# KlrShaK/opencv-SimpleSLAM

Hardware: AMD Instinct MI355X
Metric: frames/sec ALIKED+LightGlue @1241x376 (higher is better)
Workload: dtype f32 (contractions: f16 hi/lo split operands, f32 accumulate; 3 MFMA per product, 2 in attention's P.V = precision 'f16x3p1', the default since r05: profiles/r05_flip_soak.md, r06_flip_soak.md); 1 GPU; C2/C4: synthetic 1241x376x3 uint8 frame stream, ALIKED-n16 extract + LightGlue match (t-1,t), 2048 kpts/frame, min_conf 0.7, random-init weights; inputs resident in HBM before the timed region, features and matches left on the device (the `pcie` leg times the same pipeline with per-round H2D of the frames and D2H of {count, pairs}); max_kpts=2048, lightglue_layers_executed=9, pairs_per_lightglue_launch=8, frames_per_aliked_launch=8

## Files before the change

opencv-simpleslam_amd/csrc/al_plan.hpp:

```cpp
#pragma once
#include <algorithm>
#include <cstddef>
#include <cstdio>

namespace sslam {

constexpr int AL_LONG_SIDE = 1024;
constexpr int AL_PAD_DIV = 32;
constexpr int MAX_FRAMES = 16;
constexpr int B1_SW = 30;
constexpr int B2_SW = 30;
constexpr int DCN3_CS = 1;
constexpr int DCN4_CS = 4;
constexpr int AGG_PRE = 13;
constexpr int ST_W = 32, ST_H = 8;
constexpr int NHALO = 10;
constexpr int NW_R = 48, NW_OW = 64 - 2 * NHALO, NW_OH = NW_R - 2 * NHALO;
constexpr int HBINS = 4096;
constexpr int COLLECT_PPT = 16;
constexpr int SEL_CAP = 8192;
constexpr int EDGE_CAP = 2048;
constexpr int CAND_CAP = 1024 * 1024;
constexpr int REFINE_KPB = 32;
constexpr int SDDH_KSPLIT = 4;

constexpr int al_cdiv(int a, int b) { return (a + b - 1) / b; }

struct Dims {
    int H, W, C;
    int h, w;
    int Hp, Wp;
    int pl, pt;
};

enum class ALAggTile { T64x64, T64x128 };

struct ALPlan {
    int F, KF;
    int blur, ky, kx;
    float sy, sx;
    Dims d;
    int to_float_gx, pad_gx;
    int b1_strips, b1_nblk, b1_hs, b1_nb;
    int b2_strips, b2_nblk, b2_hs, b2_nb, b2_waves, b2_gx;
    int H2, W2, HW2, H3, W3, HW3, H4, W4, HW4;
    int pool3_gx, pool4_gx;
    int off3_gx, dcn3_gx, off4_gx, dcn4_gx;
    float mo3, mo4, mo;
    int gate2_gx, gate3_gx, gate4_gx, gate34_gx;
    float sy2, sx2, sy8, sx8, sy32, sx32;
    int agg_pre_gx;
    int tail_gx, tail_gy;
    int nbx, nby, n_tiles, nms_gx;
    int npx, collect_gx;
    ALAggTile agg_tile;
    float scale_x, scale_y;
};

inline ALPlan al_plan(int H, int W, int C, int F) {
    ALPlan p{};
    p.F = F; p.KF = SDDH_KSPLIT * F;
    Dims& d = p.d;
    d.H = H; d.W = W; d.C = C;
    const double ar = (double)W / (double)H;
    if (ar > 1.0) { d.h = (int)(AL_LONG_SIDE / ar); d.w = AL_LONG_SIDE; }
    else { d.h = AL_LONG_SIDE; d.w = (int)(AL_LONG_SIDE * ar); }
    const double fy = (double)H / d.h, fx = (double)W / d.w;
    p.blur = (fy > fx ? fy : fx) > 1.0;
    const double sgy = (fy - 1.0) / 2.0 > 0.001 ? (fy - 1.0) / 2.0 : 0.001, sgx = (fx - 1.0) / 2.0 > 0.001 ? (fx - 1.0) / 2.0 : 0.001;
    p.sy = (float)sgy; p.sx = (float)sgx;
    const double ksy = 2.0 * 2 * sgy, ksx = 2.0 * 2 * sgx;
    p.ky = (int)(ksy > 3 ? ksy : 3); p.kx = (int)(ksx > 3 ? ksx : 3);
    if (p.ky % 2 == 0) ++p.ky;
    if (p.kx % 2 == 0) ++p.kx;
    const int pad_h = (((d.h / AL_PAD_DIV) + 1) * AL_PAD_DIV - d.h) % AL_PAD_DIV;
    const int pad_w = (((d.w / AL_PAD_DIV) + 1) * AL_PAD_DIV - d.w) % AL_PAD_DIV;
    d.Hp = d.h + pad_h; d.Wp = d.w + pad_w; d.pl = pad_w / 2; d.pt = pad_h / 2;
    const int Hp = d.Hp, Wp = d.Wp;

// ... 10 lines not shown
    p.b2_waves = p.b2_strips * p.b2_nb * F;
    p.b2_gx = al_cdiv(p.b2_waves, 4);
    p.H3 = Hp / 8; p.W3 = Wp / 8; p.HW3 = p.H3 * p.W3;
    p.H4 = Hp / 32; p.W4 = Wp / 32; p.HW4 = p.H4 * p.W4;
    p.pool3_gx = al_cdiv(32 * p.HW3, 256); p.pool4_gx = al_cdiv(64 * p.HW4, 256);
    p.off3_gx = al_cdiv(p.W3, 32); p.dcn3_gx = DCN3_CS * al_cdiv(p.W3, 32);
    p.off4_gx = al_cdiv(p.W4, 32); p.dcn4_gx = DCN4_CS * al_cdiv(p.W4, 32);
    p.mo3 = (float)(p.H3 > p.W3 ? p.H3 : p.W3) / 4.0f;
    p.mo4 = (float)(p.H4 > p.W4 ? p.H4 : p.W4) / 4.0f;
    p.gate2_gx = al_cdiv(p.HW2, 256); p.gate3_gx = al_cdiv(32 * p.HW3, 256); p.gate4_gx = al_cdiv(32 * p.HW4, 256);
    p.gate34_gx = p.gate3_gx + p.gate4_gx;
    auto step = [](int full, int S) { return (float)(full / S - 1) / (float)(full - 1); };
    p.sy2 = step(Hp, 2); p.sx2 = step(Wp, 2); p.sy8 = step(Hp, 8); p.sx8 = step(Wp, 8);
    p.sy32 = step(Hp, 32); p.sx32 = step(Wp, 32);
    p.agg_pre_gx = al_cdiv(p.HW2 + p.HW3 + p.HW4, 256);
    p.tail_gx = al_cdiv(Wp, ST_W); p.tail_gy = al_cdiv(Hp, ST_H);
    p.nbx = al_cdiv(d.w, NW_OW); p.nby = al_cdiv(d.h, NW_OH); p.n_tiles = p.nbx * p.nby;
    p.nms_gx = al_cdiv(p.n_tiles, 4);
    p.npx = d.h * d.w;
    p.collect_gx = al_cdiv(p.npx, 256 * COLLECT_PPT);
    p.mo = (float)(d.h > d.w ? d.h : d.w) / 4.0f;
    p.agg_tile = F >= 4 ? ALAggTile::T64x128 : ALAggTile::T64x64;
    p.scale_x = (float)d.w / (float)W; p.scale_y = (float)d.h / (float)H;
    return p;
}

enum class ALRefusal { None, Size, Frames, Blur };
inline ALRefusal al_refusal(const ALPlan& p, int Hp_cap, int Wp_cap, int max_frames, char* msg, size_t n) {
    const Dims& d = p.d;
    if (!(d.Hp <= Hp_cap && d.Wp <= Wp_cap && d.h >= 8 && d.w >= 8)) {
        snprintf(msg, n, "sslam_aliked: network size %dx%d outside the instance capacity %dx%d", d.Hp, d.Wp, Hp_cap, Wp_cap);
        return ALRefusal::Size;
    }
    if (!(p.F >= 1 && p.F <= max_frames)) {
        snprintf(msg, n, "sslam_aliked: %d frames, instance capacity %d", p.F, max_frames);
        return ALRefusal::Frames;
    }
    if (!(p.kx <= 31 && p.ky <= 31)) {
        snprintf(msg, n, "sslam_aliked: blur kernel too large (%d,%d)", p.kx, p.ky);
        return ALRefusal::Blur;
    }
    return ALRefusal::None;
}

struct ALKptPlan {
    int NK;
// ... 55 lines not shown
```

opencv-simpleslam_amd/csrc/aliked_kernels.hip:

```cpp
#include "common.hpp"
#include "al_plan.hpp"
#include "gemm_f32.hpp"
#include <type_traits>
#include "gemm_f16x3.hpp"

namespace {

using sslam::f32x16;
using sslam::acc_row;
using sslam::GemmSmem;
using sslam::GemmA;
using sslam::gemm_mainloop;
using sslam::Dims;
using sslam::MAX_FRAMES; using sslam::B1_SW; using sslam::B2_SW; using sslam::DCN3_CS; using sslam::DCN4_CS; using sslam::AGG_PRE;
using sslam::ST_W; using sslam::ST_H; using sslam::NHALO; using sslam::NW_R; using sslam::NW_OW; using sslam::NW_OH; using sslam::HBINS;
using sslam::COLLECT_PPT; using sslam::SEL_CAP; using sslam::EDGE_CAP; using sslam::REFINE_KPB; using sslam::SDDH_KSPLIT;

constexpr float SELU_SCALE = 1.0507009873554804934193349852946f;
constexpr float SELU_ALPHA = 1.6732632423543772848170429916717f;
__device__ __forceinline__ float selu(float x) {
    return SELU_SCALE * (x > 0.0f ? x : SELU_ALPHA * (__expf(x) - 1.0f));
}

__device__ __forceinline__ float selu_precise(float x) {
// ... 22 lines not shown
    using B = std::conditional_t<std::is_const_v<T>, const char, char>;
    return reinterpret_cast<T*>(reinterpret_cast<B*>(p) + (size_t)f * fs);
}
struct Tile3 { int x, y, z; };
__device__ __forceinline__ Tile3 xcd_band() {
    const unsigned nx = gridDim.x, ny = gridDim.y, per = nx * ny;
    if ((per & 7u) == 0u) {
        const unsigned L = blockIdx.x + nx * blockIdx.y;
        const unsigned g = (L & 7u) * (per >> 3) + (L >> 3);
        return Tile3{(int)(g % nx), (int)(g / nx), (int)blockIdx.z};
    }
    return Tile3{(int)blockIdx.x, (int)blockIdx.y, (int)blockIdx.z};
}
template <typename T> __device__ __forceinline__ T* fsh0(T* p, int f, size_t fs) {
    return p ? fsh(p, f, fs) : nullptr;
}
template <typename T> __device__ __forceinline__ T& at_b(T* base, unsigned byte_off) {
    using B = std::conditional_t<std::is_const_v<T>, const char, char>;
    return *reinterpret_cast<T*>(reinterpret_cast<B*>(base) + byte_off);
}
struct FrameIn { const uint8_t* img[MAX_FRAMES]; };
struct FrameOut { float* xy[MAX_FRAMES]; float* desc[MAX_FRAMES]; float* score[MAX_FRAMES]; int32_t* n[MAX_FRAMES]; };

__global__ void al_to_float_kernel(FrameIn srcs, float* __restrict__ dst, Dims d,
                                   const float* __restrict__ gx, int kx, int blur, size_t fs) {
    const uint8_t* __restrict__ src = srcs.img[blockIdx.z];
    dst = fsh(dst, blockIdx.z, fs);
    const int x = blockIdx.x * blockDim.x + threadIdx.x, y = blockIdx.y;
    if (x >= d.W) return;
#pragma unroll
    for (int c = 0; c < 3; ++c) {
        const int sc = d.C == 1 ? 0 : 2 - c;
        float v;
        if (!blur) {
            v = (float)src[((size_t)y * d.W + x) * d.C + sc] / 255.0f;
        } else {
            v = 0.0f;
            const int r = kx / 2;
#pragma unroll 8
            for (int k = 0; k < kx; ++k) {
                int xx = x + k - r;
                xx = xx < 0 ? -xx : (xx >= d.W ? 2 * d.W - 2 - xx : xx);
                v += gx[k] * ((float)src[((size_t)y * d.W + xx) * d.C + sc] / 255.0f);
            }
        }
        dst[((size_t)c * d.H + y) * d.W + x] = v;
    }
}

__global__ void al_resize_pad_kernel(const float* __restrict__ src, float* __restrict__ img, Dims d,
                                     const float* __restrict__ gy, int ky, int blur, size_t fs) {
    const Tile3 tb = xcd_band();
    src = fsh(src, tb.z, fs); img = fsh(img, tb.z, fs);
    const int xp = tb.x * blockDim.x + threadIdx.x, yp = tb.y;
    if (xp >= d.Wp) return;
    const int y = min(max(yp - d.pt, 0), d.h - 1), x = min(max(xp - d.pl, 0), d.w - 1);
    const float sy_ = (float)d.H / (float)d.h, sx_ = (float)d.W / (float)d.w;
    float fy = sy_ * ((float)y + 0.5f) - 0.5f, fx = sx_ * ((float)x + 0.5f) - 0.5f;
    fy = fy < 0.0f ? 0.0f : fy;
    fx = fx < 0.0f ? 0.0f : fx;
    const int y0 = (int)fy, x0 = (int)fx;
    const int y1 = y0 + (y0 < d.H - 1), x1 = x0 + (x0 < d.W - 1);
    const float ly = fy - (float)y0, lx = fx - (float)x0, hy = 1.0f - ly, hx = 1.0f - lx;
#pragma unroll
    for (int c = 0; c < 3; ++c) {
        const float* p = src + (size_t)c * d.H * d.W;
        float v00, v01, v10, v11;
        if (!blur) {
            v00 = p[(size_t)y0 * d.W + x0]; v01 = p[(size_t)y0 * d.W + x1];
            v10 = p[(size_t)y1 * d.W + x0]; v11 = p[(size_t)y1 * d.W + x1];
        } else {
            v00 = v01 = v10 = v11 = 0.0f;
            const int r = ky / 2;
#pragma unroll 4
            for (int k = 0; k < ky; ++k) {
                int ya = y0 + k - r, yb = y1 + k - r;
                ya = ya < 0 ? -ya : (ya >= d.H ? 2 * d.H - 2 - ya : ya);
                yb = yb < 0 ? -yb : (yb >= d.H ? 2 * d.H - 2 - yb : yb);
                const float g = gy[k];
                v00 += g * p[(size_t)ya * d.W + x0]; v01 += g * p[(size_t)ya * d.W + x1];
                v10 += g * p[(size_t)yb * d.W + x0]; v11 += g * p[(size_t)yb * d.W + x1];
            }
        }
        img[((size_t)c * d.Hp + yp) * d.Wp + xp] = hy * (hx * v00 + lx * v01) + ly * (hx * v10 + lx * v11);
    }
}

typedef float f32x4 __attribute__((ext_vector_type(4)));

__global__ void al_conv16_wfrag_kernel(const float* __restrict__ w , _Float16* __restrict__ wf, int* range_flag) {
    const int i = blockIdx.x * blockDim.x + threadIdx.x;
    if (i >= 5 * 64 * 8) return;
    const int e = i & 7, lane = (i >> 3) & 63, ks = i >> 9;
    const int kk = lane >> 4, co = lane & 15, tap = 2 * ks + (kk >> 1), ci = 8 * (kk & 1) + e;
    const float v = tap < 9 ? w[(ci * 9 + tap) * 16 + co] : 0.0f;
    _Float16 hi, lo;
    al_split_weight(v, hi, lo, range_flag);
    wf[((ks * 2 + 0) * 64 + lane) * 8 + e] = hi;
    wf[((ks * 2 + 1) * 64 + lane) * 8 + e] = lo;
}


__global__ void al_conv32p_wfrag_kernel(const float* __restrict__ w , const float* __restrict__ wd ,
                                        _Float16* __restrict__ wf, int* range_flag) {
    const int i = blockIdx.x * blockDim.x + threadIdx.x;
    if (i >= 10 * 64 * 8) return;
    const int e = i & 7, lane = (i >> 3) & 63, ks = i >> 9;
// ... 787 lines not shown
    return fmaf(t.w10, top, __fmul_rn(t.w11, bot));
}
__device__ __forceinline__ float up_eval_cl32(const float* __restrict__ p, const UpTap& t, unsigned cb) {
    return up_mix(t, at_b(p, (unsigned)t.o00 * 128u + cb), at_b(p, (unsigned)t.o01 * 128u + cb),
                  at_b(p, (unsigned)t.o10 * 128u + cb), at_b(p, (unsigned)t.o11 * 128u + cb));
}
__device__ __forceinline__ float2 feat_pair32(const Pyr& P, const float* __restrict__ rnorm, int pl, int pt,
                                              int y, int x, int lane) {
    const int yp = y + pt, xp = x + pl;
    const unsigned pix = (unsigned)(yp * P.Wp + xp);
    float a, b;
    const unsigned cb = 4u * (lane & 31);
    if (lane < 32) {
        a = at_b(P.g1cl, pix * 128u + cb);
        b = up_eval_cl32(P.g3cl, up_tap(yp, xp, P.Hp, P.Wp, 8, P.sy8, P.sx8), cb);
    } else {
        a = up_eval_cl32(P.g2cl, up_tap(yp, xp, P.Hp, P.Wp, 2, P.sy2, P.sx2), cb);
        b = up_eval_cl32(P.g4cl, up_tap(yp, xp, P.Hp, P.Wp, 32, P.sy32, P.sx32), cb);
    }
    const float r = rnorm[pix];
    return make_float2(a * r, b * r);
}

__global__ __launch_bounds__(256) void al_score_tail_kernel(const float* __restrict__ s8, int Hp, int Wp,
                                                            const float* __restrict__ w2 ,
                                                            const float* __restrict__ w4 ,
                                                            const float* __restrict__ w6 ,
                                                            float* __restrict__ score, int h, int w, int pl,
                                                            int pt, size_t fs) {
    const Tile3 tb = xcd_band();
    s8 = fsh(s8, tb.z, fs); score = fsh(score, tb.z, fs);
    __shared__ float t0[8][ST_H + 6][ST_W + 6];
    __shared__ float t1[4][ST_H + 4][ST_W + 4];
    __shared__ float t2[4][ST_H + 2][ST_W + 2];
    const int x0 = tb.x * ST_W, y0 = tb.y * ST_H;
    const size_t HW = (size_t)Hp * Wp;
    for (int i = threadIdx.x; i < 8 * (ST_H + 6) * (ST_W + 6); i += 256) {
        const int c = i / ((ST_H + 6) * (ST_W + 6)), rem = i % ((ST_H + 6) * (ST_W + 6));
        const int yy = y0 + rem / (ST_W + 6) - 3, xx = x0 + rem % (ST_W + 6) - 3;
        (&t0[0][0][0])[i] = (yy >= 0 && yy < Hp && xx >= 0 && xx < Wp) ? s8[c * HW + (size_t)yy * Wp + xx] : 0.0f;
    }
    __syncthreads();
    for (int i = threadIdx.x; i < (ST_H + 4) * (ST_W + 4); i += 256) {
        const int ly = i / (ST_W + 4), lx = i % (ST_W + 4);
        const int yy = y0 + ly - 2, xx = x0 + lx - 2;
        float a[4] = {0, 0, 0, 0};
        if (yy >= 0 && yy < Hp && xx >= 0 && xx < Wp) {
#pragma unroll 1
            for (int ci = 0; ci < 8; ++ci)
#pragma unroll
                for (int tap = 0; tap < 9; ++tap) {
                    const float v = t0[ci][ly + tap / 3][lx + tap % 3];
#pragma unroll
                    for (int o = 0; o < 4; ++o) a[o] = fmaf(v, w2[(ci * 9 + tap) * 4 + o], a[o]);
                }
            for (int o = 0; o < 4; ++o) a[o] = selu(a[o]);
        }
        for (int o = 0; o < 4; ++o) t1[o][ly][lx] = a[o];
    }
    __syncthreads();
    for (int i = threadIdx.x; i < (ST_H + 2) * (ST_W + 2); i += 256) {
        const int ly = i / (ST_W + 2), lx = i % (ST_W + 2);
        const int yy = y0 + ly - 1, xx = x0 + lx - 1;
        float a[4] = {0, 0, 0, 0};
        if (yy >= 0 && yy < Hp && xx >= 0 && xx < Wp) {
#pragma unroll 1
            for (int ci = 0; ci < 4; ++ci)
#pragma unroll
                for (int tap = 0; tap < 9; ++tap) {
                    const float v = t1[ci][ly + tap / 3][lx + tap % 3];
#pragma unroll
                    for (int o = 0; o < 4; ++o) a[o] = fmaf(v, w4[(ci * 9 + tap) * 4 + o], a[o]);
                }
            for (int o = 0; o < 4; ++o) a[o] = selu(a[o]);
        }
        for (int o = 0; o < 4; ++o) t2[o][ly][lx] = a[o];
    }
    __syncthreads();
    for (int i = threadIdx.x; i < ST_H * ST_W; i += 256) {
        const int lx = i & (ST_W - 1), ly = i / ST_W;
        const int yy = y0 + ly, xx = x0 + lx;
        float a = 0.0f;
        for (int ci = 0; ci < 4; ++ci)
            for (int tap = 0; tap < 9; ++tap) a = fmaf(t2[ci][ly + tap / 3][lx + tap % 3], w6[ci * 9 + tap], a);
        const int uy = yy - pt, ux = xx - pl;
        if (uy >= 0 && uy < h && ux >= 0 && ux < w) score[(size_t)uy * w + ux] = 1.0f / (1.0f + expf(-a));
    }
}

static_assert(NW_R <= 64 && NW_OH > 0, "a column's rows are the bits of one 64-bit word");

__device__ __forceinline__ unsigned nw_up(unsigned v) { return (unsigned)__builtin_amdgcn_update_dpp(0, (int)v, 0x138, 0xf, 0xf, true); }
__device__ __forceinline__ unsigned nw_dn(unsigned v) { return (unsigned)__builtin_amdgcn_update_dpp(0, (int)v, 0x130, 0xf, 0xf, true); }
__device__ __forceinline__ float nw_up(float v) { return __builtin_bit_cast(float, nw_up(__builtin_bit_cast(unsigned, v))); }
__device__ __forceinline__ float nw_dn(float v) { return __builtin_bit_cast(float, nw_dn(__builtin_bit_cast(unsigned, v))); }
__device__ __forceinline__ float nw_row5(float v) {
    const float l1 = fmaxf(v, nw_up(v)), l2 = fmaxf(l1, nw_up(l1));
    const float r1 = fmaxf(v, nw_dn(v)), r2 = fmaxf(r1, nw_dn(r1));
    return fmaxf(l2, r2);
}
__device__ __forceinline__ void nw_pool5(const float (&in)[NW_R], float (&v)[NW_R]) {
    float hrow[NW_R], p[NW_R], q[NW_R];
#pragma unroll
    for (int y = 0; y < NW_R; ++y) hrow[y] = nw_row5(in[y]);
#pragma unroll
    for (int y = 0; y + 1 < NW_R; ++y) p[y] = fmaxf(hrow[y], hrow[y + 1]);
#pragma unroll
    for (int y = 0; y + 3 < NW_R; ++y) q[y] = fmaxf(p[y], p[y + 2]);
// ... 605 lines not shown

struct ALConvW { const float *w, *a, *b; };
struct ALDcnW { const float *ow, *ob, *w, *a, *b; };

struct sslam_aliked {
    sslam_ctx* ctx = nullptr;
    int max_h = 0, max_w = 0, max_kpts = 0;
    int max_frames = 1;
    size_t fs = 0;
    int Hp_cap = 0, Wp_cap = 0;
    sslam::OwnedSlab slab;
    float* blob = nullptr;
    ALConvW b1c1, b1c2, b2c1, b2c2;
    const float *b2dw, *b2db;
    ALDcnW b3c1, b3c2, b4c1, b4c2;
    const float *b3dw, *b3db, *b4dw, *b4db;
    _Float16 *b3c1of, *b3c2of, *b4c1of, *b4c2of;
    _Float16 *b3c1f, *b3c2f, *b4c1f, *b4c2f;
    const float *gw1, *gw2, *gw3, *gw4;
    const float *sh0, *sh2, *sh4, *sh6;
    const float *d_ow, *d_ob, *d_w2, *d_b2, *d_sf, *d_agg;
    ALCtrl* ctrl;
    uint8_t* in_u8;
    float *fsrc, *img, *x1, *x2, *p3, *off, *t3, *x3, *p4, *t4, *x4, *g2, *g3, *g4;
    float *s8, *rnorm, *score, *nms, *bsum, *gk, *g1cl, *g2cl, *g3cl, *g4cl, *pre2, *pre3, *pre4;
    unsigned long long* cand;
    unsigned* hist;
    int cand_cap;
    int* kp_index;
    int* range_sticky;
    unsigned long long* sel_keys;
    float *kp_norm, *kp_score, *patch, *h32, *pos, *sampled, *feats, *raw;
    _Float16 *d_sf_s, *d_agg_s;
    _Float16* b2c2f;
    _Float16* b1c2f;
    _Float16* b2c1f;
    float *p3cl, *t3cl, *p4cl, *t4cl;
    float *out_xy, *out_desc, *out_score;
    int32_t* out_n;
    Dims last{};
    sslam::ALKptPlan kp{};
    bool use_graphs = false;
    sslam::GraphCache graphs;
};

namespace {

// ... 11 lines not shown
    g->b2c1 = conv(16, 32); g->b2c2 = conv(32, 32); g->b2dw = take(16 * 32); g->b2db = take(32);
    g->b3c1 = dcn(32, 64); g->b3c2 = dcn(64, 64); g->b3dw = take(32 * 64); g->b3db = take(64);
    g->b4c1 = dcn(64, 128); g->b4c2 = dcn(128, 128); g->b4dw = take(64 * 128); g->b4db = take(128);
    g->gw1 = take(16 * 32); g->gw2 = take(32 * 32); g->gw3 = take(64 * 32); g->gw4 = take(128 * 32);
    g->sh0 = take(128 * 8); g->sh2 = take(8 * 9 * 4); g->sh4 = take(4 * 9 * 4); g->sh6 = take(4 * 9);
    g->d_ow = take(32 * 1152); g->d_ob = take(32); g->d_w2 = take(32 * 32); g->d_b2 = take(32);
    g->d_sf = take(128 * 128); g->d_agg = take((size_t)128 * 2048);
    SSLAM_REQUIRE(off == n_floats, "sslam_aliked_create: weight blob has %zu floats, expected %zu", n_floats, off);
    return 0;
}

constexpr int SEL_LDS = (SEL_CAP + EDGE_CAP) * 8;

int al_enqueue(sslam_aliked* g, const sslam::ALPlan& p, const FrameIn& srcs, int n_limit, const FrameOut& outs) {
    hipStream_t s = g->ctx->stream;
    (void)hipGetLastError();
    const Dims& d = p.d;
    const sslam::ALKptPlan& k = g->kp;
    const int F = p.F, KF = p.KF, NK = k.NK;
    const size_t fs = g->fs;
    const dim3 b256(256);
    hipLaunchKernelGGL(al_reset_kernel, dim3(F), b256, 0, s, g->ctrl, g->hist, fs, g->gk, p.kx, p.sx, p.ky, p.sy);

    hipLaunchKernelGGL(al_to_float_kernel, dim3(p.to_float_gx, d.H, F), b256, 0, s, srcs, g->fsrc, d, g->gk, p.kx, p.blur, fs);
    hipLaunchKernelGGL(al_resize_pad_kernel, dim3(p.pad_gx, d.Hp, F), b256, 0, s, g->fsrc, g->img, d, g->gk + 32, p.ky, p.blur, fs);
    hipLaunchKernelGGL(al_block1_rows_kernel, dim3(p.b1_strips, p.b1_nb, F), dim3(64), 0, s, g->img, g->x1, d.Hp, d.Wp, p.b1_hs,
                       g->b1c1.w, g->b1c1.a, g->b1c1.b, g->b1c2f, g->b1c2.a, g->b1c2.b, g->ctrl, fs);
    hipLaunchKernelGGL(al_block2_rows_kernel, dim3(p.b2_gx), b256, B2_LDS, s, g->x1, g->x2, p.H2, p.W2, p.b2_hs, p.b2_nb, p.b2_strips,
                       p.b2_waves, g->b2c1f, g->b2c2f, g->b2c1.a, g->b2c1.b, g->b2db, g->b2c2.a, g->b2c2.b, g->ctrl, fs);
    const dim3 off3 = dim3(p.off3_gx, p.H3, F), dcn3 = dim3(p.dcn3_gx, p.H3, F);
    hipLaunchKernelGGL(al_avgpool_kernel, dim3(p.pool3_gx, F), b256, 0, s, g->x2, g->p3, 32, p.H2, p.W2, 4, fs, g->p3cl);
    hipLaunchKernelGGL((al_offset_conv_h_kernel<32>), off3, b256, 0, s, g->p3cl, g->off, p.H3, p.W3, g->b3c1of, g->b3c1.ob, p.mo3, g->ctrl, fs);
    hipLaunchKernelGGL((al_dcn_h_kernel<32, 64, 0, DCN3_CS>), dcn3, b256, 0, s, g->p3cl, g->off, nullptr, p.H3, p.W3, g->b3c1f, g->b3c1.b, nullptr, g->t3, g->t3cl, g->ctrl, fs);
    hipLaunchKernelGGL((al_offset_conv_h_kernel<64>), off3, b256, 0, s, g->t3cl, g->off, p.H3, p.W3, g->b3c2of, g->b3c2.ob, p.mo3, g->ctrl, fs);
    hipLaunchKernelGGL((al_dcn_h_kernel<64, 64, 32, DCN3_CS>), dcn3, b256, 0, s, g->t3cl, g->off, g->p3cl, p.H3, p.W3, g->b3c2f, g->b3c2.b, g->b3db, g->x3, nullptr, g->ctrl, fs);
    const dim3 off4 = dim3(p.off4_gx, p.H4, F), dcn4 = dim3(p.dcn4_gx, p.H4, F);
    sslam::graph_cut(s);
    hipLaunchKernelGGL(al_avgpool_kernel, dim3(p.pool4_gx, F), b256, 0, s, g->x3, g->p4, 64, p.H3, p.W3, 4, fs, g->p4cl);
    hipLaunchKernelGGL((al_offset_conv_h_kernel<64>), off4, b256, 0, s, g->p4cl, g->off, p.H4, p.W4, g->b4c1of, g->b4c1.ob, p.mo4, g->ctrl, fs);
    hipLaunchKernelGGL((al_dcn_h_kernel<64, 128, 0, DCN4_CS>), dcn4, b256, 0, s, g->p4cl, g->off, nullptr, p.H4, p.W4, g->b4c1f, g->b4c1.b, nullptr, g->t4, g->t4cl, g->ctrl, fs);
    hipLaunchKernelGGL((al_offset_conv_h_kernel<128>), off4, b256, 0, s, g->t4cl, g->off, p.H4, p.W4, g->b4c2of, g->b4c2.ob, p.mo4, g->ctrl, fs);
    hipLaunchKernelGGL((al_dcn_h_kernel<128, 128, 64, DCN4_CS>), dcn4, b256, 0, s, g->t4cl, g->off, g->p4cl, p.H4, p.W4, g->b4c2f, g->b4c2.b, g->b4db, g->x4, nullptr, g->ctrl, fs);
    hipLaunchKernelGGL(al_gate_kernel<32>, dim3(p.gate2_gx, F), b256, 0, s, g->x2, g->g2, p.HW2, g->gw2, g->g2cl, fs);
    hipLaunchKernelGGL(al_gate_small_kernel, dim3(p.gate34_gx, F), b256, 0, s, GateSmall{g->x3, g->g3, 64, p.HW3, g->gw3, g->g3cl},
                       GateSmall{g->x4, g->g4, 128, p.HW4, g->gw4, g->g4cl}, p.gate3_gx, fs);
    Pyr P{g->x1, g->g2, g->g3, g->g4, g->gw1, d.Hp, d.Wp, g->g1cl};
    P.sy2 = p.sy2; P.sx2 = p.sx2; P.sy8 = p.sy8; P.sx8 = p.sx8; P.sy32 = p.sy32; P.sx32 = p.sx32;
    P.g2cl = g->g2cl; P.g3cl = g->g3cl; P.g4cl = g->g4cl;
    P.pre2 = g->pre2; P.pre3 = g->pre3; P.pre4 = g->pre4;
    hipLaunchKernelGGL(al_agg_pre_kernel, dim3(p.agg_pre_gx, F), b256, 0, s, g->g2, g->g3, g->g4, g->sh0, g->pre2, g->pre3, g->pre4,
                       d.Hp, d.Wp, fs);
    hipLaunchKernelGGL(al_aggregate_kernel, dim3(p.pad_gx, d.Hp, F), b256, 0, s, P, g->sh0, g->s8, g->rnorm, fs);
    hipLaunchKernelGGL(al_score_tail_kernel, dim3(p.tail_gx, p.tail_gy, F), b256, 0, s, g->s8, d.Hp, d.Wp, g->sh2, g->sh4, g->sh6,
                       g->score, d.h, d.w, d.pl, d.pt, fs);
    hipLaunchKernelGGL(al_nms_wave_kernel, dim3(p.nms_gx, F), b256, 0, s, g->score, d.h, d.w, p.nbx, p.n_tiles, g->nms, g->bsum, 0.2f,
                       g->cand, g->cand_cap, g->ctrl, g->hist, fs);
    sslam::graph_cut(s);
    hipLaunchKernelGGL(al_collect_kernel, dim3(p.collect_gx, F), b256, 0, s, g->nms, p.npx, 0.0f, 1, g->bsum, p.n_tiles, g->cand,
                       g->cand_cap, g->ctrl, g->hist, fs);
    hipLaunchKernelGGL(al_select_kernel, dim3(F), dim3(1024), SEL_LDS, s, g->cand, g->cand_cap, n_limit, g->sel_keys, g->ctrl, g->hist, fs);
    hipLaunchKernelGGL(al_refine_kernel, dim3(k.refine_gx, F), b256, 0, s, g->score, d.h, d.w, g->sel_keys, g->kp_index, g->kp_norm,
                       g->kp_score, g->ctrl, fs);
    hipLaunchKernelGGL(al_patch_kernel, dim3(k.patch_gx, F), b256, 0, s, P, g->rnorm, d.pl, d.pt, d.h, d.w, g->kp_norm, g->patch, g->ctrl, fs);
    hipLaunchKernelGGL((al_gemm_kernel<64, 64, 1, 1>), dim3(1, k.rows64, KF), b256, 0, s, g->patch, 1152, g->d_ow, nullptr, 32, g->h32,
                       1, NK, 0, g->ctrl, SDDH_KSPLIT, fs);
    hipLaunchKernelGGL(al_offsets_kernel, dim3(k.offsets_gx, F), b256, 0, s, g->h32, NK, g->d_ob, g->d_w2, g->d_b2, g->kp_norm, d.h, d.w,
                       p.mo, g->pos, g->ctrl, fs);
    _Float16* sampled_h = reinterpret_cast<_Float16*>(g->sampled);
    _Float16* feats_h = reinterpret_cast<_Float16*>(g->feats);
    hipLaunchKernelGGL(al_sample_kernel, dim3(k.sample_gx, F), b256, 0, s, P, g->rnorm, d.pl, d.pt, d.h, d.w, g->pos, sampled_h,
                       k.plane, g->ctrl, fs);
    hipLaunchKernelGGL((al_gemm_h_kernel<64, 128, 1, 2, true>), dim3(1, k.rows64_x16, F), b256, 0, s, sampled_h, k.plane, 128, g->d_sf_s,
                       (size_t)128 * 128, 128, nullptr, feats_h, k.plane, 16, k.rows_x16, g->ctrl, 1, fs);
    if (p.agg_tile == sslam::ALAggTile::T64x128)
        hipLaunchKernelGGL((al_gemm_h_kernel<64, 128, 1, 2, false>), dim3(1, k.rows64, KF), b256, 0, s, feats_h, k.plane, 2048,
                           g->d_agg_s, (size_t)128 * 2048, 128, g->raw, nullptr, 0, 1, NK, g->ctrl, SDDH_KSPLIT, fs);
// ... 35 lines not shown
                  SEL_CAP);
    SSLAM_HIP_CHECK(hipSetDevice(ctx->device));
    std::unique_ptr<sslam_aliked> g(new sslam_aliked());
    g->ctx = ctx; g->max_h = max_h; g->max_w = max_w; g->max_kpts = max_kpts; g->max_frames = max_frames;
    g->kp = sslam::al_kpt_plan(max_kpts);
    g->Hp_cap = sslam::AL_LONG_SIDE + sslam::AL_PAD_DIV; g->Wp_cap = sslam::AL_LONG_SIDE + sslam::AL_PAD_DIV;
    const sslam::ALExtents e = sslam::al_extents((size_t)g->Hp_cap * g->Wp_cap, (size_t)max_h * max_w, (size_t)max_kpts);
    g->cand_cap = sslam::CAND_CAP;
    auto bind_shared = [&](sslam::Slab& A) {
        g->blob = A.take<float>(n_floats);
        g->d_sf_s = A.take<_Float16>(2 * 128 * 128); g->d_agg_s = A.take<_Float16>((size_t)2 * 128 * 2048);
        g->b2c2f = A.take<_Float16>(2 * 32 * 288);
        g->b1c2f = A.take<_Float16>(5 * 2 * 64 * 8);
        g->b2c1f = A.take<_Float16>(10 * 2 * 64 * 8);
        g->b3c1f = A.take<_Float16>((size_t)(9 * 2 + 0) * 2 * 2 * 512); g->b3c2f = A.take<_Float16>((size_t)(9 * 4 + 2) * 2 * 2 * 512);
        g->b4c1f = A.take<_Float16>((size_t)(9 * 4 + 0) * 4 * 2 * 512); g->b4c2f = A.take<_Float16>((size_t)(9 * 8 + 4) * 4 * 2 * 512);
        g->b3c1of = A.take<_Float16>(18 * 2 * 512); g->b3c2of = A.take<_Float16>(36 * 2 * 512); g->b4c1of = A.take<_Float16>(36 * 2 * 512); g->b4c2of = A.take<_Float16>(72 * 2 * 512);
        g->gk = A.take<float>(64);
        g->range_sticky = A.take<int>(4);
    };
    auto bind_frame = [&](sslam::Slab& A) {
        g->ctrl = A.take<ALCtrl>(e.ctrl);
        g->in_u8 = A.take<uint8_t>(e.in_u8);
        g->fsrc = A.take<float>(e.fsrc); g->img = A.take<float>(e.img);
        g->x1 = A.take<float>(e.x1); g->x2 = A.take<float>(e.x2);
        g->p3 = A.take<float>(e.p3); g->off = A.take<float>(e.off);
        g->t3 = A.take<float>(e.t3); g->x3 = A.take<float>(e.x3);
        g->p3cl = A.take<float>(e.p3cl); g->t3cl = A.take<float>(e.t3cl);
        g->p4cl = A.take<float>(e.p4cl); g->t4cl = A.take<float>(e.t4cl);
        g->p4 = A.take<float>(e.p4); g->t4 = A.take<float>(e.t4); g->x4 = A.take<float>(e.x4);
        g->g2 = A.take<float>(e.g2); g->g3 = A.take<float>(e.g3); g->g4 = A.take<float>(e.g4);
        g->g2cl = A.take<float>(e.g2cl); g->g3cl = A.take<float>(e.g3cl); g->g4cl = A.take<float>(e.g4cl);
        g->s8 = A.take<float>(e.s8); g->rnorm = A.take<float>(e.rnorm); g->g1cl = A.take<float>(e.g1cl);
        g->pre2 = A.take<float>(e.pre2); g->pre3 = A.take<float>(e.pre3); g->pre4 = A.take<float>(e.pre4);
        g->score = A.take<float>(e.score); g->nms = A.take<float>(e.nms); g->bsum = A.take<float>(e.bsum);
        g->cand = A.take<unsigned long long>(e.cand); g->hist = A.take<unsigned>(e.hist);
        g->kp_index = A.take<int>(e.kp_index); g->sel_keys = A.take<unsigned long long>(e.sel_keys);
        g->kp_norm = A.take<float>(e.kp_norm); g->kp_score = A.take<float>(e.kp_score);
        g->patch = A.take<float>(e.patch); g->h32 = A.take<float>(e.h32); g->pos = A.take<float>(e.pos);
        g->sampled = A.take<float>(e.sampled); g->feats = A.take<float>(e.feats);
        g->raw = A.take<float>(e.raw);
        g->out_xy = A.take<float>(e.out_xy); g->out_desc = A.take<float>(e.out_desc); g->out_score = A.take<float>(e.out_score);
        g->out_n = A.take<int32_t>(e.out_n);
    };
    sslam::Slab ms, mf;
    bind_shared(ms);
    bind_frame(mf);
// ... 192 lines not shown
```

Baseline: 1223 frames/s.

## Fuse u8-to-float blur and resize-pad into one LDS-tiled preprocess kernel; restage score tail

Replaces the separate to_float and resize_pad kernels with one tiled kernel. It stages raw uint8 rows into LDS with dword loads, applies the horizontal blur through a byte-to-float lookup table, then does the vertical blur and bilinear resize from LDS. This removes the full-resolution float intermediate (fsrc) and one launch. The score tail kernel is also reworked: LDS buffers are flattened and aliased, staging is a lane per column, and each thread computes two adjacent outputs with float2 window reads. The risks are LDS pressure from the dynamic tile size and more complex edge handling.

Result: faster. 1242 frames/s, median of 6 (+1.6%).

```diff
diff --git a/opencv-simpleslam_amd/csrc/al_plan.hpp b/opencv-simpleslam_amd/csrc/al_plan.hpp
--- a/opencv-simpleslam_amd/csrc/al_plan.hpp
+++ b/opencv-simpleslam_amd/csrc/al_plan.hpp
@@ -14,6 +14,7 @@
 constexpr int DCN4_CS = 4;
 constexpr int AGG_PRE = 13;
 constexpr int ST_W = 32, ST_H = 8;
+constexpr int PRE_LDS_MAX = 48 * 1024;
 constexpr int NHALO = 10;
 constexpr int NW_R = 48, NW_OW = 64 - 2 * NHALO, NW_OH = NW_R - 2 * NHALO;
 constexpr int HBINS = 4096;
@@ -55,6 +56,7 @@
     int npx, collect_gx;
     ALAggTile agg_tile;
     float scale_x, scale_y;
+    int pre_tw, pre_th, pre_gx, pre_gy, pre_cols, pre_rows, pre_raw, pre_lds;
 };
 
 inline ALPlan al_plan(int H, int W, int C, int F) {
@@ -111,6 +113,19 @@
     p.mo = (float)(d.h > d.w ? d.h : d.w) / 4.0f;
     p.agg_tile = F >= 4 ? ALAggTile::T64x128 : ALAggTile::T64x64;
     p.scale_x = (float)d.w / (float)W; p.scale_y = (float)d.h / (float)H;
+    {
+        static constexpr int ladder[][2] = {{64, 8}, {32, 8}, {32, 4}, {16, 4}, {16, 2}, {8, 2}, {8, 1}, {4, 1}};
+        const int rx = p.blur ? p.kx / 2 : 0, ry = p.blur ? p.ky / 2 : 0, planes = C == 1 ? 1 : 3;
+        for (const auto& t : ladder) {
+            p.pre_tw = t[0]; p.pre_th = t[1];
+            p.pre_cols = (int)(fx * (t[0] - 1)) + 4;
+            p.pre_rows = (int)(fy * (t[1] - 1)) + 4 + 2 * ry;
+            p.pre_raw = ((p.pre_cols + 2 * rx) * C + 3) / 4 * 4 + 4;
+            p.pre_lds = 256 * 4 + planes * p.pre_rows * p.pre_cols * 4 + p.pre_rows * p.pre_raw;
+            if (p.pre_lds <= PRE_LDS_MAX) break;
+        }
+        p.pre_gx = al_cdiv(Wp, p.pre_tw); p.pre_gy = al_cdiv(Hp, p.pre_th);
+    }
     return p;
 }
 
diff --git a/opencv-simpleslam_amd/csrc/aliked_kernels.hip b/opencv-simpleslam_amd/csrc/aliked_kernels.hip
--- a/opencv-simpleslam_amd/csrc/aliked_kernels.hip
+++ b/opencv-simpleslam_amd/csrc/aliked_kernels.hip
@@ -68,67 +68,150 @@
 struct FrameIn { const uint8_t* img[MAX_FRAMES]; };
 struct FrameOut { float* xy[MAX_FRAMES]; float* desc[MAX_FRAMES]; float* score[MAX_FRAMES]; int32_t* n[MAX_FRAMES]; };
 
-__global__ void al_to_float_kernel(FrameIn srcs, float* __restrict__ dst, Dims d,
-                                   const float* __restrict__ gx, int kx, int blur, size_t fs) {
-    const uint8_t* __restrict__ src = srcs.img[blockIdx.z];
-    dst = fsh(dst, blockIdx.z, fs);
-    const int x = blockIdx.x * blockDim.x + threadIdx.x, y = blockIdx.y;
-    if (x >= d.W) return;
-#pragma unroll
-    for (int c = 0; c < 3; ++c) {
-        const int sc = d.C == 1 ? 0 : 2 - c;
-        float v;
-        if (!blur) {
-            v = (float)src[((size_t)y * d.W + x) * d.C + sc] / 255.0f;
-        } else {
-            v = 0.0f;
-            const int r = kx / 2;
-#pragma unroll 8
-            for (int k = 0; k < kx; ++k) {
-                int xx = x + k - r;
-                xx = xx < 0 ? -xx : (xx >= d.W ? 2 * d.W - 2 - xx : xx);
-                v += gx[k] * ((float)src[((size_t)y * d.W + xx) * d.C + sc] / 255.0f);
+struct PreTile { int tw, th, cols, rows, raw; };
+__device__ __forceinline__ int al_reflect(int i, int n) {
+    i = i < 0 ? -i : (i >= n ? 2 * n - 2 - i : i);
+    return min(max(i, 0), n - 1);
+}
+__device__ __forceinline__ void al_src_pos(int o, int n_in, float s, int& i0, int& i1, float& l) {
+    float f = fmaf(s, __fadd_rn((float)o, 0.5f), -0.5f);
+    f = f < 0.0f ? 0.0f : f;
+    i0 = (int)f; i1 = i0 + (i0 < n_in - 1); l = __fsub_rn(f, (float)i0);
+}
+__global__ __launch_bounds__(256) void al_preprocess_kernel(FrameIn srcs, float* __restrict__ img, Dims d, const float* __restrict__ gk,
+                                                            int kx, int ky, int blur, PreTile t, size_t fs) {
+    extern __shared__ __attribute__((aligned(16))) unsigned char pre_lds[];
+    const Tile3 tb = xcd_band();
+    const uint8_t* __restrict__ src = srcs.img[tb.z];
+    img = fsh(img, tb.z, fs);
+    const int planes = d.C == 1 ? 1 : 3;
+    float* tab = reinterpret_cast<float*>(pre_lds);
+    float* hb = tab + 256;
+    uint8_t* raw = reinterpret_cast<uint8_t*>(hb + planes * t.rows * t.cols);
+    const int tid = threadIdx.x, lane = tid & 63, wv = tid >> 6;
+    const float sy_ = (float)d.H / (float)d.h, sx_ = (float)d.W / (float)d.w;
+    const int rx = blur ? kx / 2 : 0, ry = blur ? ky / 2 : 0;
+    const int xp_a = tb.x * t.tw, yp_a = tb.y * t.th;
+    const int xp_b = min(xp_a + t.tw, d.Wp) - 1, yp_b = min(yp_a + t.th, d.Hp) - 1;
+    int xlo, xhi, ylo, yhi, unused; float unused_l;
+    al_src_pos(min(max(xp_a - d.pl, 0), d.w - 1), d.W, sx_, xlo, unused, unused_l);
+    al_src_pos(min(max(xp_b - d.pl, 0), d.w - 1), d.W, sx_, unused, xhi, unused_l);
+    al_src_pos(min(max(yp_a - d.pt, 0), d.h - 1), d.H, sy_, ylo, unused, unused_l);
+    al_src_pos(min(max(yp_b - d.pt, 0), d.h - 1), d.H, sy_, unused, yhi, unused_l);
+    ylo -= ry; yhi += ry;
+    const int ncols = min(xhi - xlo + 1, t.cols), nrows = min(yhi - ylo + 1, t.rows);
+    const int rlo = max(xlo - rx, 0), rhi = min(xhi + rx, d.W - 1);
+    const int raw_bytes = (rhi - rlo + 1) * d.C;
+    const uint8_t* const src_end = src + (size_t)d.H * d.W * d.C;
+
+    tab[tid] = (float)tid / 255.0f;
+    for (int j = wv; j < nrows; j += 4) {
+        const uint8_t* p = src + ((size_t)al_reflect(ylo + j, d.H) * d.W + rlo) * d.C;
+        const int shift = (int)(reinterpret_cast<uintptr_t>(p) & 3u);
+        p -= shift;
+        const int ndw = min((shift + raw_bytes + 3) >> 2, t.raw >> 2);
+        uint32_t* row = reinterpret_cast<uint32_t*>(raw + j * t.raw);
+        for (int i = lane; i < ndw; i += 64) {
+            const uint8_t* q = p + 4 * i;
+            uint32_t v;
+            if (q >= src && q + 4 <= src_end) {
+                v = *reinterpret_cast<const uint32_t*>(q);
+            } else {
+                v = 0;
+                for (int b = 0; b < 4; ++b)
+                    if (q + b >= src && q + b < src_end) v |= (uint32_t)q[b] << (8 * b);
             }
-        }
-        dst[((size_t)c * d.H + y) * d.W + x] = v;
-    }
-}
-
-__global__ void al_resize_pad_kernel(const float* __restrict__ src, float* __restrict__ img, Dims d,
-                                     const float* __restrict__ gy, int ky, int blur, size_t fs) {
-    const Tile3 tb = xcd_band();
-    src = fsh(src, tb.z, fs); img = fsh(img, tb.z, fs);
-    const int xp = tb.x * blockDim.x + threadIdx.x, yp = tb.y;
-    if (xp >= d.Wp) return;
-    const int y = min(max(yp - d.pt, 0), d.h - 1), x = min(max(xp - d.pl, 0), d.w - 1);
-    const float sy_ = (float)d.H / (float)d.h, sx_ = (float)d.W / (float)d.w;
-    float fy = sy_ * ((float)y + 0.5f) - 0.5f, fx = sx_ * ((float)x + 0.5f) - 0.5f;
-    fy = fy < 0.0f ? 0.0f : fy;
-    fx = fx < 0.0f ? 0.0f : fx;
-    const int y0 = (int)fy, x0 = (int)fx;
-    const int y1 = y0 + (y0 < d.H - 1), x1 = x0 + (x0 < d.W - 1);
-    const float ly = fy - (float)y0, lx = fx - (float)x0, hy = 1.0f - ly, hx = 1.0f - lx;
-#pragma unroll
-    for (int c = 0; c < 3; ++c) {
-        const float* p = src + (size_t)c * d.H * d.W;
-        float v00, v01, v10, v11;
-        if (!blur) {
-            v00 = p[(size_t)y0 * d.W + x0]; v01 = p[(size_t)y0 * d.W + x1];
-            v10 = p[(size_t)y1 * d.W + x0]; v11 = p[(size_t)y1 * d.W + x1];
-        } else {
-            v00 = v01 = v10 = v11 = 0.0f;
-            const int r = ky / 2;
+            row[i] = v;
+        }
+    }
+    __syncthreads();
+    {
+        const float* __restrict__ gx = gk;
+        const int step_j = 256 / ncols, step_i = 256 - step_j * ncols;
+        int j = tid / ncols, i = tid - j * ncols;
+        const unsigned src_lo = (unsigned)reinterpret_cast<uintptr_t>(src);
+        const int plane = t.rows * t.cols;
+        while (j < nrows) {
+            const unsigned shift = (src_lo + (unsigned)((al_reflect(ylo + j, d.H) * d.W + rlo) * d.C)) & 3u;
+            const uint8_t* row = raw + j * t.raw + shift - rlo * d.C;
+            float* o = hb + j * t.cols + i;
+            const int x = xlo + i;
+            if (planes == 1) {
+                float v = 0.0f;
+                if (!blur) v = tab[row[x * d.C]];
+                else
 #pragma unroll 4
-            for (int k = 0; k < ky; ++k) {
-                int ya = y0 + k - r, yb = y1 + k - r;
-                ya = ya < 0 ? -ya : (ya >= d.H ? 2 * d.H - 2 - ya : ya);
-                yb = yb < 0 ? -yb : (yb >= d.H ? 2 * d.H - 2 - yb : yb);
-                const float g = gy[k];
-                v00 += g * p[(size_t)ya * d.W + x0]; v01 += g * p[(size_t)ya * d.W + x1];
-                v10 += g * p[(size_t)yb * d.W + x0]; v11 += g * p[(size_t)yb * d.W + x1];
+                    for (int k = 0; k < kx; ++k) v = fmaf(gx[k], tab[row[min(max(al_reflect(x + k - rx, d.W), rlo), rhi) * d.C]], v);
+                o[0] = v;
+            } else {
+                float v0 = 0.0f, v1 = 0.0f, v2 = 0.0f;
+                if (!blur) {
+                    const uint8_t* px = row + x * d.C;
+                    v0 = tab[px[2]]; v1 = tab[px[1]]; v2 = tab[px[0]];
+                } else {
+#pragma unroll 4
+                    for (int k = 0; k < kx; ++k) {
+                        const uint8_t* px = row + min(max(al_reflect(x + k - rx, d.W), rlo), rhi) * d.C;
+                        const float g = gx[k];
+                        v0 = fmaf(g, tab[px[2]], v0); v1 = fmaf(g, tab[px[1]], v1); v2 = fmaf(g, tab[px[0]], v2);
+                    }
+                }
+                o[0] = v0; o[plane] = v1; o[2 * plane] = v2;
             }
-        }
-        img[((size_t)c * d.Hp + yp) * d.Wp + xp] = hy * (hx * v00 + lx * v01) + ly * (hx * v10 + lx * v11);
+            j += step_j; i += step_i;
+            if (i >= ncols) { i -= ncols; ++j; }
+        }
+    }
+    __syncthreads();
+    {
+        const float* __restrict__ gy = gk + 32;
+        const int sh = __ffs(t.tw) - 1, xp = xp_a + (tid & (t.tw - 1));
+        if (xp >= d.Wp) return;
+        int x0, x1; float lx;
+        al_src_pos(min(max(xp - d.pl, 0), d.w - 1), d.W, sx_, x0, x1, lx);
+        const float hx = __fsub_rn(1.0f, lx);
+        const bool dx = x1 != x0;
+        x0 -= xlo;
+        for (int ty = tid >> sh; ty < t.th; ty += 256 >> sh) {
+            const int yp = yp_a + ty;
+            if (yp >= d.Hp) break;
+            int y0, y1; float ly;
+            al_src_pos(min(max(yp - d.pt, 0), d.h - 1), d.H, sy_, y0, y1, ly);
+            const float hy = __fsub_rn(1.0f, ly);
+            const bool dy = y1 != y0;
+            const float* p = hb + (y0 - ylo - ry) * t.cols + x0;
+            float out = 0.0f;
+#pragma unroll
+            for (int c = 0; c < 3; ++c) {
+                if (c == 0 || planes == 3) {
+                    const float* q = p + c * t.rows * t.cols;
+                    float a0 = q[0], a1 = q[1];
+                    a1 = dx ? a1 : a0;
+                    float v00, v01, v10, v11;
+                    if (!blur) {
+                        q += t.cols;
+                        const float n0 = q[0], n1 = q[1];
+                        v00 = a0; v01 = a1;
+                        v10 = dy ? n0 : a0; v11 = dy ? (dx ? n1 : n0) : a1;
+                    } else {
+                        v00 = v01 = v10 = v11 = 0.0f;
+#pragma unroll 4
+                        for (int k = 0; k < ky; ++k) {
+                            const float g = gy[k];
+                            q += t.cols;
+                            float n0 = q[0], n1 = q[1];
+                            n1 = dx ? n1 : n0;
+                            v00 = fmaf(g, a0, v00); v01 = fmaf(g, a1, v01);
+                            v10 = fmaf(g, dy ? n0 : a0, v10); v11 = fmaf(g, dy ? n1 : a1, v11);
+                            a0 = n0; a1 = n1;
+                        }
+                    }
+                    const float top = fmaf(lx, v01, __fmul_rn(hx, v00)), bot = fmaf(hx, v10, __fmul_rn(lx, v11));
+                    out = __fadd_rn(__fmul_rn(hy, top), __fmul_rn(ly, bot));
+                }
+                img[((size_t)c * d.Hp + yp) * d.Wp + xp] = out;
+            }
+        }
     }
 }
 
@@ -962,68 +1045,101 @@
     return make_float2(a * r, b * r);
 }
 
-__global__ __launch_bounds__(256) void al_score_tail_kernel(const float* __restrict__ s8, int Hp, int Wp,
-                                                            const float* __restrict__ w2 ,
-                                                            const float* __restrict__ w4 ,
-                                                            const float* __restrict__ w6 ,
-                                                            float* __restrict__ score, int h, int w, int pl,
-                                                            int pt, size_t fs) {
+constexpr int ST_T = 256;
+constexpr int ST_P0 = ST_W + 6, ST_R0 = ST_H + 6, ST_N0 = 8 * ST_R0 * ST_P0;
+constexpr int ST_P1 = ST_W + 4, ST_R1 = ST_H + 4, ST_N1 = 4 * ST_R1 * ST_P1;
+constexpr int ST_P2 = ST_W + 2, ST_R2 = ST_H + 2, ST_N2 = 4 * ST_R2 * ST_P2;
+static_assert(ST_P0 % 2 == 0 && ST_P1 % 2 == 0 && ST_P2 % 2 == 0 && ST_N0 % 2 == 0 && ST_N2 <= ST_N0, "8-byte window reads; t2 in t0's place");
+static_assert(ST_R1 * (ST_P1 / 2) <= ST_T && ST_R2 * (ST_P2 / 2) <= ST_T && ST_H * ST_W == ST_T, "one run per thread and layer");
+static_assert(ST_P0 <= 64 && (8 * ST_R0) % (ST_T / 64) == 0, "staging: a lane per column, the waves take the same number of rows");
+
+template <int CIN, int P>
+__device__ __forceinline__ void st_conv_run(const float* tin, int plane, const float* __restrict__ w , float (&a)[2][4]) {
+#pragma unroll 1
+    for (int ci = 0; ci < CIN; ++ci) {
+        float win[3][4];
+#pragma unroll
+        for (int dy = 0; dy < 3; ++dy) {
+            const float2 q = *reinterpret_cast<const float2*>(tin + dy * P), e = *reinterpret_cast<const float2*>(tin + dy * P + 2);
+            win[dy][0] = q.x; win[dy][1] = q.y; win[dy][2] = e.x; win[dy][3] = e.y;
+        }
+#pragma unroll
+        for (int tap = 0; tap < 9; ++tap)
+#pragma unroll
+            for (int p = 0; p < 2; ++p) {
+                const float v = win[tap / 3][p + tap % 3];
+#pragma unroll
+                for (int o = 0; o < 4; ++o) a[p][o] = fmaf(v, w[(ci * 9 + tap) * 4 + o], a[p][o]);
+            }
+        tin += plane;
+    }
+}
+
+__global__ __launch_bounds__(ST_T) void al_score_tail_kernel(const float* __restrict__ s8, int Hp, int Wp,
+                                                             const float* __restrict__ w2 ,
+                                                             const float* __restrict__ w4 ,
+                                                             const float* __restrict__ w6 ,
+                                                             float* __restrict__ score, int h, int w, int pl,
+                                                             int pt, size_t fs) {
     const Tile3 tb = xcd_band();
     s8 = fsh(s8, tb.z, fs); score = fsh(score, tb.z, fs);
-    __shared__ float t0[8][ST_H + 6][ST_W + 6];
-    __shared__ float t1[4][ST_H + 4][ST_W + 4];
-    __shared__ float t2[4][ST_H + 2][ST_W + 2];
+    __shared__ __attribute__((aligned(16))) float lds[ST_N0 + ST_N1];
+    float* const t0 = lds;
+    float* const t1 = lds + ST_N0;
+    float* const t2 = lds;
     const int x0 = tb.x * ST_W, y0 = tb.y * ST_H;
+    const int tid = threadIdx.x;
     const size_t HW = (size_t)Hp * Wp;
-    for (int i = threadIdx.x; i < 8 * (ST_H + 6) * (ST_W + 6); i += 256) {
-        const int c = i / ((ST_H + 6) * (ST_W + 6)), rem = i % ((ST_H + 6) * (ST_W + 6));
-        const int yy = y0 + rem / (ST_W + 6) - 3, xx = x0 + rem % (ST_W + 6) - 3;
-        (&t0[0][0][0])[i] = (yy >= 0 && yy < Hp && xx >= 0 && xx < Wp) ? s8[c * HW + (size_t)yy * Wp + xx] : 0.0f;
+    if ((tid & 63) < ST_P0) {
+        const int wv = __builtin_amdgcn_readfirstlane(tid >> 6), lane = tid & 63;
+        const int xx = x0 + lane - 3;
+        const bool xin = xx >= 0 && xx < Wp;
+        const unsigned xb = 4u * (unsigned)min(max(xx, 0), Wp - 1);
+#pragma unroll
+        for (int r = 0; r < 8 * ST_R0 / (ST_T / 64); ++r) {
+            const int row = (ST_T / 64) * r + wv, c = row / ST_R0, yy = y0 + row - c * ST_R0 - 3;
+            const float* rowp = s8 + c * HW + (size_t)min(max(yy, 0), Hp - 1) * Wp;
+            const float v = at_b(rowp, xb);
+            t0[row * ST_P0 + lane] = (xin && yy >= 0 && yy < Hp) ? v : 0.0f;
+        }
     }
     __syncthreads();
-    for (int i = threadIdx.x; i < (ST_H + 4) * (ST_W + 4); i += 256) {
-        const int ly = i / (ST_W + 4), lx = i % (ST_W + 4);
-        const int yy = y0 + ly - 2, xx = x0 + lx - 2;
-        float a[4] = {0, 0, 0, 0};
-        if (yy >= 0 && yy < Hp && xx >= 0 && xx < Wp) {
-#pragma unroll 1
-            for (int ci = 0; ci < 8; ++ci)
-#pragma unroll
-                for (int tap = 0; tap < 9; ++tap) {
-                    const float v = t0[ci][ly + tap / 3][lx + tap % 3];
-#pragma unroll
-                    for (int o = 0; o < 4; ++o) a[o] = fmaf(v, w2[(ci * 9 + tap) * 4 + o], a[o]);
-                }
-            for (int o = 0; o < 4; ++o) a[o] = selu(a[o]);
-        }
-        for (int o = 0; o < 4; ++o) t1[o][ly][lx] = a[o];
+    {
+        constexpr int RUNS = ST_P1 / 2;
+        const int ly = tid / RUNS, lx = (tid - ly * RUNS) * 2;
+        if (tid < ST_R1 * RUNS) {
+            float a[2][4] = {};
+            st_conv_run<8, ST_P0>(t0 + ly * ST_P0 + lx, ST_R0 * ST_P0, w2, a);
+            const int yy = y0 + ly - 2, xx = x0 + lx - 2;
+            const bool yin = yy >= 0 && yy < Hp, in0 = yin && xx >= 0 && xx < Wp, in1 = yin && xx + 1 >= 0 && xx + 1 < Wp;
+#pragma unroll
+            for (int o = 0; o < 4; ++o)
+                *reinterpret_cast<float2*>(t1 + (o * ST_R1 + ly) * ST_P1 + lx) =
+                    make_float2(in0 ? selu(a[0][o]) : 0.0f, in1 ? selu(a[1][o]) : 0.0f);
+        }
     }
     __syncthreads();
-    for (int i = threadIdx.x; i < (ST_H + 2) * (ST_W + 2); i += 256) {
-        const int ly = i / (ST_W + 2), lx = i % (ST_W + 2);
-        const int yy = y0 + ly - 1, xx = x0 + lx - 1;
-        float a[4] = {0, 0, 0, 0};
-        if (yy >= 0 && yy < Hp && xx >= 0 && xx < Wp) {
-#pragma unroll 1
-            for (int ci = 0; ci < 4; ++ci)
-#pragma unroll
-                for (int tap = 0; tap < 9; ++tap) {
-                    const float v = t1[ci][ly + tap / 3][lx + tap % 3];
-#pragma unroll
-                    for (int o = 0; o < 4; ++o) a[o] = fmaf(v, w4[(ci * 9 + tap) * 4 + o], a[o]);
-                }
-            for (int o = 0; o < 4; ++o) a[o] = selu(a[o]);
-        }
-        for (int o = 0; o < 4; ++o) t2[o][ly][lx] = a[o];
+    {
+        constexpr int RUNS = ST_P2 / 2;
+        const int ly = tid / RUNS, lx = (tid - ly * RUNS) * 2;
+        if (tid < ST_R2 * RUNS) {
+            float a[2][4] = {};
+            st_conv_run<4, ST_P1>(t1 + ly * ST_P1 + lx, ST_R1 * ST_P1, w4, a);
+            const int yy = y0 + ly - 1, xx = x0 + lx - 1;
+            const bool yin = yy >= 0 && yy < Hp, in0 = yin && xx >= 0 && xx < Wp, in1 = yin && xx + 1 >= 0 && xx + 1 < Wp;
+#pragma unroll
+            for (int o = 0; o < 4; ++o)
+                *reinterpret_cast<float2*>(t2 + (o * ST_R2 + ly) * ST_P2 + lx) =
+                    make_float2(in0 ? selu(a[0][o]) : 0.0f, in1 ? selu(a[1][o]) : 0.0f);
+        }
     }
     __syncthreads();
-    for (int i = threadIdx.x; i < ST_H * ST_W; i += 256) {
-        const int lx = i & (ST_W - 1), ly = i / ST_W;
-        const int yy = y0 + ly, xx = x0 + lx;
+    {
+        const int lx = tid & (ST_W - 1), ly = tid / ST_W;
         float a = 0.0f;
         for (int ci = 0; ci < 4; ++ci)
-            for (int tap = 0; tap < 9; ++tap) a = fmaf(t2[ci][ly + tap / 3][lx + tap % 3], w6[ci * 9 + tap], a);
-        const int uy = yy - pt, ux = xx - pl;
+            for (int tap = 0; tap < 9; ++tap) a = fmaf(t2[(ci * ST_R2 + ly + tap / 3) * ST_P2 + lx + tap % 3], w6[ci * 9 + tap], a);
+        const int uy = y0 + ly - pt, ux = x0 + lx - pl;
         if (uy >= 0 && uy < h && ux >= 0 && ux < w) score[(size_t)uy * w + ux] = 1.0f / (1.0f + expf(-a));
     }
 }
@@ -1675,7 +1791,7 @@
     const float *d_ow, *d_ob, *d_w2, *d_b2, *d_sf, *d_agg;
     ALCtrl* ctrl;
     uint8_t* in_u8;
-    float *fsrc, *img, *x1, *x2, *p3, *off, *t3, *x3, *p4, *t4, *x4, *g2, *g3, *g4;
+    float *img, *x1, *x2, *p3, *off, *t3, *x3, *p4, *t4, *x4, *g2, *g3, *g4;
     float *s8, *rnorm, *score, *nms, *bsum, *gk, *g1cl, *g2cl, *g3cl, *g4cl, *pre2, *pre3, *pre4;
     unsigned long long* cand;
     unsigned* hist;
@@ -1733,8 +1849,8 @@
     const dim3 b256(256);
     hipLaunchKernelGGL(al_reset_kernel, dim3(F), b256, 0, s, g->ctrl, g->hist, fs, g->gk, p.kx, p.sx, p.ky, p.sy);
 
-    hipLaunchKernelGGL(al_to_float_kernel, dim3(p.to_float_gx, d.H, F), b256, 0, s, srcs, g->fsrc, d, g->gk, p.kx, p.blur, fs);
-    hipLaunchKernelGGL(al_resize_pad_kernel, dim3(p.pad_gx, d.Hp, F), b256, 0, s, g->fsrc, g->img, d, g->gk + 32, p.ky, p.blur, fs);
+    hipLaunchKernelGGL(al_preprocess_kernel, dim3(p.pre_gx, p.pre_gy, F), b256, (size_t)p.pre_lds, s, srcs, g->img, d, g->gk, p.kx, p.ky,
+                       p.blur, PreTile{p.pre_tw, p.pre_th, p.pre_cols, p.pre_rows, p.pre_raw}, fs);
     hipLaunchKernelGGL(al_block1_rows_kernel, dim3(p.b1_strips, p.b1_nb, F), dim3(64), 0, s, g->img, g->x1, d.Hp, d.Wp, p.b1_hs,
                        g->b1c1.w, g->b1c1.a, g->b1c1.b, g->b1c2f, g->b1c2.a, g->b1c2.b, g->ctrl, fs);
     hipLaunchKernelGGL(al_block2_rows_kernel, dim3(p.b2_gx), b256, B2_LDS, s, g->x1, g->x2, p.H2, p.W2, p.b2_hs, p.b2_nb, p.b2_strips,
@@ -1762,7 +1878,7 @@
     hipLaunchKernelGGL(al_agg_pre_kernel, dim3(p.agg_pre_gx, F), b256, 0, s, g->g2, g->g3, g->g4, g->sh0, g->pre2, g->pre3, g->pre4,
                        d.Hp, d.Wp, fs);
     hipLaunchKernelGGL(al_aggregate_kernel, dim3(p.pad_gx, d.Hp, F), b256, 0, s, P, g->sh0, g->s8, g->rnorm, fs);
-    hipLaunchKernelGGL(al_score_tail_kernel, dim3(p.tail_gx, p.tail_gy, F), b256, 0, s, g->s8, d.Hp, d.Wp, g->sh2, g->sh4, g->sh6,
+    hipLaunchKernelGGL(al_score_tail_kernel, dim3(p.tail_gx, p.tail_gy, F), dim3(ST_T), 0, s, g->s8, d.Hp, d.Wp, g->sh2, g->sh4, g->sh6,
                        g->score, d.h, d.w, d.pl, d.pt, fs);
     hipLaunchKernelGGL(al_nms_wave_kernel, dim3(p.nms_gx, F), b256, 0, s, g->score, d.h, d.w, p.nbx, p.n_tiles, g->nms, g->bsum, 0.2f,
                        g->cand, g->cand_cap, g->ctrl, g->hist, fs);
@@ -1844,7 +1960,7 @@
     auto bind_frame = [&](sslam::Slab& A) {
         g->ctrl = A.take<ALCtrl>(e.ctrl);
         g->in_u8 = A.take<uint8_t>(e.in_u8);
-        g->fsrc = A.take<float>(e.fsrc); g->img = A.take<float>(e.img);
+        g->img = A.take<float>(e.img);
         g->x1 = A.take<float>(e.x1); g->x2 = A.take<float>(e.x2);
         g->p3 = A.take<float>(e.p3); g->off = A.take<float>(e.off);
         g->t3 = A.take<float>(e.t3); g->x3 = A.take<float>(e.x3);
```
